# DCDmllm/AnyEdit

Measured on AMD Instinct MI355X. Metric: edited-images/sec @512x512, 50 DDIM steps, higher is better.
Workload: dtype bf16; 1 GPU; configs[1]: AnySD (SD-1.5 UNet in=8 + task embedding/expert adapters) 512x512 bf16, 50 DDIM steps, batch=4/GPU, 3-branch CFG (UNet batch 12); images_per_gpu=4, ddim_steps=50, cfg_branches=3, hip_graph=True, parallelism=dp1 (image-sharded, no data-path collective)

## Files before the change

anyedit_amd/_lib.py:

```python
import ctypes
import os

import torch

_HERE = os.path.dirname(os.path.abspath(__file__))
LIB_PATH = os.environ.get("AE_LIB_PATH") or os.path.join(_HERE, "libanyedit_hip.so")

c_void_p, c_int, c_long, c_float = ctypes.c_void_p, ctypes.c_int, ctypes.c_long, ctypes.c_float

SIGNATURES = {
    "ae_version": [],
    "ae_last_error": [],
    "ae_device_arch": [ctypes.c_char_p, c_int],
    "ae_device_info": [ctypes.POINTER(c_int), ctypes.POINTER(c_long), ctypes.POINTER(c_int)],
    "ae_gemm_bf16": [c_void_p, c_long, c_void_p, c_long, c_int, c_void_p, c_long, c_void_p, c_long, c_int, c_int, c_int,
                     c_void_p, c_void_p, c_long, c_void_p, c_long, c_int, c_int, c_int, c_void_p, c_void_p],
    "ae_conv3x3_workspace_floats": [c_int, c_int, c_int, c_int, c_int, c_int, c_int],
    "ae_conv3x3_bf16": [c_void_p, c_void_p, c_void_p, c_void_p, c_long, c_void_p, c_void_p, c_int, c_int, c_int, c_int, c_int,
                        c_int, c_int, c_int, c_void_p, c_void_p, c_int, c_void_p],
    "ae_conv3x3_up2_bf16": [c_void_p, c_void_p, c_void_p, c_void_p, c_int, c_int, c_int, c_int, c_int, c_void_p, c_void_p],
    "ae_gemm_plan": [c_int] * 8 + [ctypes.POINTER(c_int)],
    "ae_conv3x3_plan": [c_int] * 11 + [ctypes.POINTER(c_int)],
    "ae_conv3x3_up2_plan": [c_int] * 6 + [ctypes.POINTER(c_int)],
    "ae_groupnorm_rows_per_chunk": [c_int, c_int],
# ... 86 lines not shown
    "ae_clip_embed_bf16": [c_void_p, c_int, c_void_p, c_void_p, c_void_p, c_int, c_int, c_int, c_int, c_int, c_void_p],
    "ae_bias_act_f32_bf16": [c_void_p, c_long, c_void_p, c_void_p, c_long, c_long, c_int, c_int, c_void_p],
    "ae_clip_pool_eos_bf16": [c_void_p, c_int, c_void_p, c_void_p, c_int, c_int, c_int, c_long, c_void_p],
    "ae_clip_patch_rows_bf16": [c_void_p, c_int, c_void_p, c_int, c_int, c_int, c_int, c_int, c_int, c_float, c_void_p, c_void_p, c_void_p],
    "ae_clip_vision_embed_ln_bf16": [c_void_p, c_long, c_void_p, c_void_p, c_void_p, c_void_p, c_void_p, c_int, c_int, c_int, c_float, c_void_p],
    "ae_clip_vision_pool_ln_bf16": [c_void_p, c_long, c_void_p, c_void_p, c_void_p, c_int, c_int, c_float, c_void_p],
    "ae_dino_embed_bf16": [c_void_p, c_long, c_void_p, c_void_p, c_void_p, c_void_p, c_int, c_int, c_int, c_void_p],
    "ae_swiglu_f32_bf16": [c_void_p, c_long, c_void_p, c_void_p, c_long, c_long, c_int, c_void_p],
    "ae_swin_window_attn_bf16": [c_void_p, c_long, c_void_p, c_void_p, c_void_p, c_long, c_int, c_int, c_int, c_int, c_int, c_int, c_int, c_float, c_void_p],
    "ae_swin_merge_ln_bf16": [c_void_p, c_void_p, c_void_p, c_void_p, c_int, c_int, c_int, c_int, c_float, c_void_p],
    "ae_scale_residual_f32_bf16": [c_void_p, c_long, c_void_p, c_void_p, c_void_p, c_long, c_void_p, c_long, c_long, c_int, c_void_p],
    "ae_biattn_split_rows": [c_int],
    "ae_biattn_workspace_bytes": [c_int, c_int, c_int, c_int, c_int],
    "ae_biattn_bf16": [c_void_p, c_long] * 4 + [c_void_p, c_void_p] + [c_void_p, c_long] * 2 + [c_int] * 5 + [c_float, c_void_p, c_long, c_void_p],
    "ae_attn_masked_short_bf16": [c_void_p] * 5 + [c_int] * 4 + [c_long] * 12 + [c_float, c_void_p],
    "ae_contrastive_bf16": [c_void_p, c_long, c_void_p, c_void_p, c_void_p, c_long, c_void_p] + [c_int] * 5 + [c_void_p],
    "ae_topk_rows_max_n": [],
    "ae_topk_rows_f32": [c_void_p, c_long, c_void_p, c_int, c_int, c_int, c_void_p],
    "ae_gdino_proposals_f32": [c_void_p, ctypes.POINTER(c_int), ctypes.POINTER(c_int), c_int, c_void_p, c_void_p, c_int, c_int, c_void_p],
    "ae_gdino_query_sine": [c_void_p, c_void_p, c_void_p, c_void_p, c_long, c_int, c_int, c_int, c_void_p],
    "ae_gdino_box_refine_f32": [c_void_p, c_long, c_void_p, c_void_p, c_void_p, c_void_p, c_void_p, c_long, c_int, c_void_p],
    "ae_gdino_text_spans": [c_void_p, c_int, c_int, c_int, c_int] + [c_long] * 8 + [c_void_p, c_void_p, c_void_p, c_void_p],
    "ae_bert_embed_ln_bf16": [c_void_p, c_void_p, c_void_p] + [c_void_p] * 6 + [c_int] * 6 + [c_float, c_void_p],
    "ae_attn_span_short_bf16": [c_void_p] * 5 + [c_int] * 4 + [c_long] * 12 + [c_float, c_void_p],
    "ae_gdino_level_geometry": [c_void_p, c_int, c_int, c_int, ctypes.POINTER(c_int), ctypes.POINTER(c_int), c_int, c_float, c_float, c_void_p, c_void_p, c_void_p,
                                c_void_p, c_int, c_void_p],
    "ae_gdino_neck_groupnorm_workspace_floats": [c_int, c_int],
    "ae_gdino_neck_groupnorm": [c_void_p, c_long, c_void_p, c_void_p, c_float, c_void_p, c_long, c_long, c_int, c_int, c_void_p, c_void_p],
    "ae_gdino_ground": [c_void_p, c_void_p, c_float, c_float, c_void_p, c_void_p, c_void_p, c_void_p, c_void_p, c_int, c_int, c_int, c_void_p],
    "ae_hed_stem_bf16": [c_void_p, c_int, c_long, c_long, c_long, c_long, c_void_p, c_void_p, c_void_p, c_void_p, c_int, c_int, c_int, c_int, c_void_p],
    "ae_relu_bf16": [c_void_p, c_long, c_void_p],
    "ae_hed_tail_bf16": [c_void_p, c_void_p, c_void_p, c_void_p, c_void_p, c_int, c_int, c_int, c_int, c_void_p],
    "ae_hed_fuse": [c_void_p] * 7 + [c_int] * 4 + [c_void_p],
}
_RESTYPES = {"ae_last_error": ctypes.c_char_p, "ae_groupnorm_workspace_floats": c_long, "ae_conv3x3_workspace_floats": c_long,
             "ae_groupnorm_bwd_workspace_floats": c_long, "ae_attn_fp8_workspace_bytes": c_long, "ae_attn_bwd_workspace_floats": c_long,
             "ae_biattn_workspace_bytes": c_long, "ae_gdino_neck_groupnorm_workspace_floats": c_long}


class AnyEditHipError(RuntimeError):
    pass


def _load():
    if not os.path.exists(LIB_PATH):
        raise ImportError(
            f"{LIB_PATH} is missing: the HIP extension is REQUIRED (no CPU/eager fallback exists). "
            "Build it with `python -c 'import __graft_entry__ as g; g.build()'` or `python anyedit_amd/build.py`.")
    lib = ctypes.CDLL(LIB_PATH)
    for name, argtypes in SIGNATURES.items():
        fn = getattr(lib, name)
        fn.argtypes = argtypes
        fn.restype = _RESTYPES.get(name, c_int)
    return lib


lib = _load()


def check(rc, what=""):
    if rc != 0:
        msg = lib.ae_last_error()
        raise AnyEditHipError(f"{what} failed (rc={rc}): {msg.decode() if msg else ''}")


def device_arch():
# ... 4 lines not shown
```

anyedit_amd/build.py:

```python
import hashlib
import os
import shutil
import subprocess
import sys

HERE = os.path.dirname(os.path.abspath(__file__))
CSRC = os.path.join(HERE, "csrc")
LIB = os.path.join(HERE, "libanyedit_hip.so")
SOURCES = ["c_api.hip", "gemm_conv.hip", "gemm_rowpanel.hip", "ff_fused.hip", "attention.hip", "attention_fast.hip", "attention_fp8.hip", "attention_bwd.hip", "norm.hip", "elementwise.hip", "backward.hip", "gate.hip", "expert_kv.hip", "msda.hip",
           "sam_decoder.hip", "clip_text.hip", "clip_vision.hip", "dino_vision.hip", "swin.hip", "gdino_encoder.hip", "gdino_decoder.hip", "gdino_text.hip", "gdino_neck.hip", "hed.hip"]
EXTRA = {"gemm_conv.hip": ["-fno-slp-vectorize"], "gemm_rowpanel.hip": ["-fno-slp-vectorize"], "ff_fused.hip": ["-fno-slp-vectorize"], "attention.hip": ["-ffinite-math-only"],
         "attention_fast.hip": ["-ffinite-math-only", "-fno-slp-vectorize"], "attention_fp8.hip": ["-ffinite-math-only"],
         "attention_bwd.hip": ["-ffinite-math-only"], "clip_text.hip": ["-ffinite-math-only"]}
FLAGS = ["--offload-arch=gfx950", "-O3", "-std=c++17", "-fPIC", "-fno-gpu-rdc", "-Wno-unused-result"]


def _hipcc():
    for c in (shutil.which("hipcc"), "/opt/rocm/bin/hipcc"):
        if c and os.path.exists(c):
            return c
    raise RuntimeError("hipcc not found: the HIP extension cannot be built")


def _digest():
    h = hashlib.sha256()
    for name in sorted(os.listdir(CSRC)):
        with open(os.path.join(CSRC, name), "rb") as f:
            h.update(name.encode() + f.read())
    h.update((" ".join(FLAGS) + repr(sorted(EXTRA.items()))).encode())
    return h.hexdigest()


def build_library(force=False, verbose=True, variant=None, extra_flags=None):
    lib = LIB if variant is None else os.path.join(HERE, f"libanyedit_hip_{variant}.so")
    extra = {k: list(v) for k, v in EXTRA.items()}
    for k, v in (extra_flags or {}).items():
        if k not in SOURCES:
            raise ValueError(f"{k} is not a source of the library")
        extra[k] = extra.get(k, []) + list(v)
    stamp = lib + ".sha256"
    dig = _digest() if variant is None else None
    if not force and dig is not None and os.path.exists(lib) and os.path.exists(stamp) and open(stamp).read().strip() == dig:
        return lib
    objdir = os.path.join(HERE, "build" if variant is None else f"build_{variant}")
# ... 38 lines not shown
```

anyedit_amd/csrc/norm.hip:

```cpp
#include "common.hpp"
#include <stdlib.h>

#ifndef GN_CS_U
#define GN_CS_U 4
#endif

namespace {

constexpr int GN_MAXR = 8;

struct GNArgs {
    const bf16_t* x; const bf16_t* x2;
    int C1;
    const float* gamma; const float* beta;
    bf16_t* y;
    float* part;
    float* coef;
    int B, HW, C, groups, rows_per_chunk, nchunk, act;
    float eps;
    float* stat;
    const bf16_t* dy; bf16_t* dx; bf16_t* dx2;
    float* part2;
    float* coef2;
    int* counters;
// ... 997 lines not shown
        AE_REQUIRE(HW % 32 == 0, "ae_groupnorm_nhwc_bf16: producer statistics are kept per 32-row slab: HW=%d must be a multiple of 32", HW);
        AE_REQUIRE((x2 == nullptr) == (colstats2 == nullptr), "ae_groupnorm_nhwc_bf16: statistics are needed for both sources of a concat input");
        AE_REQUIRE(((uintptr_t)colstats & 7) == 0 && ((uintptr_t)colstats2 & 7) == 0, "ae_groupnorm_nhwc_bf16: colstats alignment");
        AE_REQUIRE((long)(HW / 32) * (C / groups) < (1L << 20), "ae_groupnorm_nhwc_bf16: %ld slab sums per group exceed the 2^20 the statistics fold indexes exactly", (long)(HW / 32) * (C / groups));
        p.cs1 = colstats; p.cs2 = colstats2;
        hipLaunchKernelGGL(gn_finalize_cs_kernel, dim3(groups, B), dim3(256), 0, s, p);
        int rc0 = ae_check_launch("ae_groupnorm_nhwc_bf16(finalize from producer statistics)");
        if (rc0) return rc0;
        hipLaunchKernelGGL(gn_apply_kernel<false>, grid, dim3(threads), 0, s, p);
        return ae_check_launch("ae_groupnorm_nhwc_bf16(apply)");
    }
    static const int slab = getenv("AE_GN_SLAB") ? atoi(getenv("AE_GN_SLAB")) : 1;
    if (slab && HW <= 256) {
        const int cpg = C / groups;
        const int gp = (cpg % 8 == 0) ? 1 : ((2 * cpg) % 8 == 0 ? 2 : ((4 * cpg) % 8 == 0 ? 4 : 0));
        bool done = false;
        if (gp == 1 && groups % 1 == 0) done = launch_gn_slab<1>(p, cpg, s);
        else if (gp == 2 && groups % 2 == 0) done = launch_gn_slab<2>(p, cpg, s);
        else if (gp == 4 && groups % 4 == 0) done = launch_gn_slab<4>(p, cpg, s);
        if (done) return ae_check_launch("ae_groupnorm_nhwc_bf16(slab)");
    }
    hipLaunchKernelGGL(gn_stats_kernel, grid, dim3(threads), (size_t)(threads / ncc) * 2 * C * sizeof(float), s, p);
    int rc = ae_check_launch("ae_groupnorm_nhwc_bf16(stats)");
    if (rc) return rc;
    if (p.counters) {
        hipLaunchKernelGGL(gn_apply_kernel<false>, grid, dim3(threads), 0, s, p);
        return ae_check_launch("ae_groupnorm_nhwc_bf16(apply)");
    }
    hipLaunchKernelGGL(gn_finalize_kernel, dim3(B), dim3(1024), 0, s, p);
    rc = ae_check_launch("ae_groupnorm_nhwc_bf16(finalize)");
    if (rc) return rc;
    hipLaunchKernelGGL(gn_apply_kernel<false>, grid, dim3(threads), 0, s, p);
    return ae_check_launch("ae_groupnorm_nhwc_bf16(apply)");
}

extern "C" int ae_layernorm_bf16(const void* x, const float* gamma, const float* beta, void* y, int M, int C, float eps,
                                 void* stream) {
    AE_REQUIRE(x && gamma && beta && y, "ae_layernorm_bf16: null pointer");
    AE_REQUIRE(M > 0 && C > 0 && C % 8 == 0, "ae_layernorm_bf16: C=%d must be a positive multiple of 8", C);
    AE_REQUIRE(C <= 4096, "ae_layernorm_bf16: C=%d > 4096 unsupported", C);
    AE_REQUIRE(((uintptr_t)x & 15) == 0 && ((uintptr_t)y & 15) == 0, "ae_layernorm_bf16: 16-byte alignment");
    dim3 grid((M + 3) / 4), block(256);
    const int ncc = C / 8;
    hipStream_t s = (hipStream_t)stream;
    static const int rows_kernel = getenv("AE_LN_ROWS") ? atoi(getenv("AE_LN_ROWS")) : 1;
    const bool al16 = (((uintptr_t)gamma | (uintptr_t)beta) & 15) == 0;
    if (rows_kernel && al16 && ncc % 5 == 0 && (ncc == 40 || ncc == 80 || ncc == 160 || ncc == 320)) {
        const int L = ncc / 5, rpb = 4 * (64 / L);
        dim3 g2((unsigned)((M + rpb - 1) / rpb));
        if (L == 8) hipLaunchKernelGGL((layernorm_rows_kernel<8, 5>), g2, block, 0, s, (const bf16_t*)x, gamma, beta, (bf16_t*)y, M, C, eps);
        else if (L == 16) hipLaunchKernelGGL((layernorm_rows_kernel<16, 5>), g2, block, 0, s, (const bf16_t*)x, gamma, beta, (bf16_t*)y, M, C, eps);
        else if (L == 32) hipLaunchKernelGGL((layernorm_rows_kernel<32, 5>), g2, block, 0, s, (const bf16_t*)x, gamma, beta, (bf16_t*)y, M, C, eps);
        else hipLaunchKernelGGL((layernorm_rows_kernel<64, 5>), g2, block, 0, s, (const bf16_t*)x, gamma, beta, (bf16_t*)y, M, C, eps);
        return ae_check_launch("ae_layernorm_bf16");
    }
    if (ncc <= 64) hipLaunchKernelGGL(layernorm_kernel<1>, grid, block, 0, s, (const bf16_t*)x, gamma, beta, (bf16_t*)y, M, C, eps);
    else if (ncc <= 128) hipLaunchKernelGGL(layernorm_kernel<2>, grid, block, 0, s, (const bf16_t*)x, gamma, beta, (bf16_t*)y, M, C, eps);
    else if (ncc <= 192) hipLaunchKernelGGL(layernorm_kernel<3>, grid, block, 0, s, (const bf16_t*)x, gamma, beta, (bf16_t*)y, M, C, eps);
    else hipLaunchKernelGGL(layernorm_kernel<8>, grid, block, 0, s, (const bf16_t*)x, gamma, beta, (bf16_t*)y, M, C, eps);
    return ae_check_launch("ae_layernorm_bf16");
}

extern "C" int ae_layernorm_window_supported(int C) {
    const int ncc = C / 8;
    return C % 8 == 0 && (ncc == 40 || ncc == 80 || ncc == 160 || ncc == 320);
}
// ... 134 lines not shown
```

anyedit_amd/ldm/modules/attention.py:

```python
import os

import torch
import torch.nn as nn

from anyedit_amd import ops
from anyedit_amd.ldm.util import default, exists
from anyedit_amd.ldm.modules.diffusionmodules.util import Linear, Conv2d, LayerNorm, checkpoint

BF16 = torch.bfloat16
_FF_TAIL = os.environ.get("AE_FF_TAIL", "1") != "0"
_SEG2_160 = os.environ.get("AE_ATTN_SEG2_160", "1") != "0"


def zero_module(module):
    for p in module.parameters():
        p.detach().zero_()
    return module


class _GN6(nn.GroupNorm):

    def _affine(self):
        if ops.cache_stale(self, "_pk", self.weight, self.bias):
            self._pk = (self.weight.detach().float().contiguous(), self.bias.detach().float().contiguous())
# ... 275 lines not shown


class SpatialTransformer(nn.Module):

    def __init__(self, in_channels, n_heads, d_head, depth=1, dropout=0., context_dim=None, disable_self_attn=False,
                 use_linear=False, use_checkpoint=True):
        super().__init__()
        if exists(context_dim) and not isinstance(context_dim, list):
            context_dim = [context_dim] * depth
        if context_dim is None:
            context_dim = [None] * depth
        self.in_channels = in_channels
        inner_dim = n_heads * d_head
        self.norm = Normalize(in_channels)
        if not use_linear:
            self.proj_in = Conv2d(in_channels, inner_dim, kernel_size=1, stride=1, padding=0)
        else:
            self.proj_in = Linear(in_channels, inner_dim)
        self.transformer_blocks = nn.ModuleList(
            [BasicTransformerBlock(inner_dim, n_heads, d_head, dropout=dropout, context_dim=context_dim[d],
                                   disable_self_attn=disable_self_attn, checkpoint=use_checkpoint) for d in range(depth)])
        if not use_linear:
            self.proj_out = zero_module(Conv2d(inner_dim, in_channels, kernel_size=1, stride=1, padding=0))
        else:
            self.proj_out = zero_module(Linear(in_channels, inner_dim))
        self.use_linear = use_linear

    def rows(self, x, B, H, W, context_rows=None, kv_cache=None, colstats=None, out_colstats=None):
        if isinstance(context_rows, (list, tuple)):
            ctxs = list(context_rows)
        else:
            ctxs = [context_rows] * len(self.transformer_blocks)
        N = H * W
        h = self.norm.rows(x, B, N, colstats=colstats)
        pin = self.proj_in._packed()
        M, Ci = h.shape[0], pin["w"].shape[0]
        st = None
        if self.transformer_blocks[0].wants_rowstats(M, Ci) and ops.ln_fold_plan(M, Ci, h.shape[1], ops.EPI_NONE, 1):
            st = ops.rowstats_buffer(M, Ci, h.device)
        h = ops.gemm(h, pin["w"], pin["b"], rowstats=st)
        pout = self.proj_out._packed()
        last = len(self.transformer_blocks) - 1
        tail_ok = self.transformer_blocks[last].takes_tail(M, Ci) and pout["w"].shape == (Ci, Ci) and x.shape[1] == Ci
        for i, blk in enumerate(self.transformer_blocks):
            tail = (pout["w"], pout["b"], x, out_colstats) if (tail_ok and i == last) else None
            h = blk.rows(h, B, N, context_rows=ctxs[i], kv_cache=kv_cache, rowstats=st if i == 0 else None, tail=tail)
        if tail_ok:
            return h
        return ops.gemm(h, pout["w"], pout["b"], residual=x, colstats=out_colstats)

    def forward(self, x, context=None):
        B, C, H, W = x.shape
        if isinstance(context, list):
            ctx = [None if c is None else c.reshape(-1, c.shape[-1]).to(BF16).contiguous() for c in context]
        else:
            ctx = None if context is None else context.reshape(-1, context.shape[-1]).to(BF16).contiguous()
        y = self.rows(ops.nchw_to_rows(x), B, H, W, context_rows=ctx)
        return ops.rows_to_nchw(y, B, H, W, out_dtype=x.dtype)
```

anyedit_amd/ops.py:

```python
import torch

import collections
import ctypes
import os
import threading

from ._lib import lib, check as _check

BF16 = torch.bfloat16
EPI_NONE, EPI_GELU, EPI_GEGLU, EPI_SILU, EPI_RELU = 0, 1, 2, 3, 4


def _s():
    return torch.cuda.current_stream().cuda_stream


def _p(t):
    return None if t is None else t.data_ptr()


_live = threading.local()


def _tmp(t):
# ... 460 lines not shown

def _gn_counters(device, B):
    if not _GN_TAIL:
        return None
    key = (device, torch.cuda.current_stream(device).cuda_stream)
    c = _GN_COUNTERS.get(key)
    if c is None or c.numel() < B:
        c = _GN_COUNTERS[key] = torch.zeros(max(B, 256), dtype=torch.int32, device=device)
    return c


def groupnorm(x, gamma, beta, B, HW, eps, silu=False, groups=32, x2=None, out=None, stat_out=None, colstats=None, colstats2=None):
    if _TAPE is not None and _TAPE.active:
        return _TAPE.groupnorm(x, gamma, beta, B, HW, eps, silu=silu, groups=groups, x2=x2, out=out)
    _chk(x, BF16, "groupnorm.x", 2)
    C1 = x.shape[1]
    C = C1 + (x2.shape[1] if x2 is not None else 0)
    if not x.is_contiguous() or (x2 is not None and not x2.is_contiguous()):
        raise ValueError("groupnorm: inputs must be contiguous")
    if out is None:
        out = torch.empty(B * HW, C, dtype=BF16, device=x.device)
    if colstats is not None and (x2 is None) != (colstats2 is None):
        colstats = colstats2 = None
    if colstats is not None:
        for t, c, n in ((colstats, C1, "colstats"), (colstats2, C - C1, "colstats2")):
            if t is not None and (t.dtype != torch.float32 or tuple(t.shape) != (B * HW // 32, c, 2) or not t.is_contiguous() or HW % 32):
                raise ValueError(f"groupnorm: {n} must be a contiguous fp32 [{B * HW // 32}, {c}, 2] buffer (HW % 32 == 0), got {tuple(t.shape)}")
    nws = int(lib.ae_groupnorm_workspace_floats(B, HW, C, groups))
    ws = torch.empty(nws, dtype=torch.float32, device=x.device)
    check(lib.ae_groupnorm_nhwc_bf16(_p(x), _p(x2), C1, _p(gamma), _p(beta), _p(out), B, HW, C, groups, eps,
                                     1 if silu else 0, _p(ws), _p(_gn_counters(x.device, B)), _p(stat_out), _p(colstats), _p(colstats2), _s()),
          "ae_groupnorm_nhwc_bf16")
    return out


def layernorm(x, gamma, beta, eps=1e-5, out=None):
    if _TAPE is not None and _TAPE.active:
        return _TAPE.layernorm(x, gamma, beta, eps=eps, out=out)
    _chk(x, BF16, "layernorm.x", 2)
    if not x.is_contiguous():
        raise ValueError("layernorm: x must be contiguous")
    M, C = x.shape
    if out is None:
        out = torch.empty_like(x)
    check(lib.ae_layernorm_bf16(_p(x), _p(gamma), _p(beta), _p(out), M, C, eps, _s()), "ae_layernorm_bf16")
    return out


def attention(q, k, v, B, H, Nq, Nk, D, scale, q_strides, k_strides, v_strides, out=None, rel_h=None, rel_w=None,
              kH=0, kW=0, key_mask=None, out_scale=None, accumulate=False, seg2=None, lse=None, lse2=None, o_strides=None):
    if _TAPE is not None and _TAPE.active:
        return _TAPE.attention(q, k, v, B, H, Nq, Nk, D, scale, q_strides, k_strides, v_strides, out=out, key_mask=key_mask,
                               out_scale=out_scale, accumulate=accumulate, seg2=seg2, rel_h=rel_h)
    if out is None:
        out = torch.empty(B, Nq, H * D, dtype=BF16, device=q.device)
    if o_strides is None:
        o_strides = (Nq * H * D, D, H * D)
    if seg2 is not None:
        k2, v2, Nk2, k2_strides, v2_strides, scale2 = seg2
        seg_args = (_p(k2), _p(v2), Nk2, *k2_strides, *v2_strides, _p(scale2))
    else:
        seg_args = (None, None, 0, 0, 0, 0, 0, 0, 0, None)
    check(lib.ae_attn_fwd_bf16(_p(q), _p(k), _p(v), _p(out), B, H, Nq, Nk, D, *q_strides, *k_strides, *v_strides, *o_strides,
                               scale, _p(rel_h), _p(rel_w), kH, kW, _p(key_mask), _p(out_scale), 1 if accumulate else 0,
                               *seg_args, _p(lse), _p(lse2), _s()), "ae_attn_fwd_bf16")
    return out
# ... 1597 lines not shown


def _gemm_ln_label(_r, a, w, bias, residual, epilogue, out, M, N, K, rowstats_out, ln_stats, nparts, ln_colsum, eps):
    nb = 2 * (M * K + N * K) + _r.numel() * 2 + (2 * M * N if residual is not None else 0)
    tag = "rowstats" if rowstats_out is not None else "LNfold"
    p = gemm_plan(M, N, K, epilogue, ln_mode=1 if rowstats_out is not None else 2)
    if p.rowpanel:
        return f"gemm_rowpanel_kernel<K=320,{tag}{',geglu' if epilogue == EPI_GEGLU else ''}>|M={M} N={N}", 2.0 * M * N * K, nb
    return f"gemm_kernel<{plan_label(p)},dense,{tag}>|M={M} N={N} K={K}", 2.0 * M * N * K, float(nb)


def _up2_label(_r, x, w4, bias, B, H, W, **_):
    y = _r[0]
    Cout, Cin = w4.shape[1], x.shape[1]
    tl = plan_label(up2_plan(B, H, W, Cin, Cout, _.get("colstats") is not None))
    nb = 2 * (x.numel() + 16 * Cin * Cout) + 2 * y.numel()
    return f"gemm_kernel<{tl},conv3x3,up2x2>|M={y.shape[0]} Cin={Cin} Cout={Cout}", 2.0 * y.shape[0] * Cout * 4 * Cin, float(nb)


conv3x3_up2 = _wrap_profiled(conv3x3_up2, _up2_label)
ff_fused = _wrap_profiled(ff_fused, lambda _r, x, gamma, beta, eps, w1, b1, w2img, b2, residual=None, out=None, w3=None, b3=None, residual3=None, colstats=None: (
    f"ff_fused_kernel<C=320{',proj_out' if w3 is not None else ''}>|M={x.shape[0]} H={w1.shape[0] // 2}",
    2.0 * x.shape[0] * x.shape[1] * (3 * (w1.shape[0] // 2) + (x.shape[1] if w3 is not None else 0)),
    float(2 * (x.numel() * (2 + (residual is not None and residual is not x) + (residual3 is not None)) + w1.numel() + w2img.numel() + (w3.numel() if w3 is not None else 0))),
    2 if colstats is not None else 1))
_ln_gemm_fused = _wrap_profiled(_ln_gemm_launch, _ln_gemm_label)
_gemm_ln_launch = _wrap_profiled(_gemm_ln_launch, _gemm_ln_label)
gemm = _wrap_profiled(gemm, _gemm_label)
attention_fp8 = _wrap_profiled(attention_fp8, _attn8_label)
conv3x3 = _wrap_profiled(conv3x3, _conv_label)
attention = _wrap_profiled(attention, _attn_label)
groupnorm = _wrap_profiled(groupnorm, _gn_label)
layernorm = _wrap_profiled(layernorm, _ln_label)
expert_kv = _wrap_profiled(expert_kv, lambda _r, x, W, experts, tokens: (
    f"expert_kv_fwd_kernel|rows={x.shape[0]} N={W.shape[1]} Dc={W.shape[2]}", 2.0 * x.shape[0] * W.shape[1] * W.shape[2], 4.0 * (x.shape[0] // tokens) * W.shape[1] * W.shape[2]))
expert_kv_dgrad = _wrap_profiled(expert_kv_dgrad, lambda _r, dy, W, experts, tokens: (
    f"expert_kv_dgrad_kernel|rows={dy.shape[0]} N={W.shape[1]} Dc={W.shape[2]}", 2.0 * dy.shape[0] * W.shape[1] * W.shape[2], 4.0 * (dy.shape[0] // tokens) * W.shape[1] * W.shape[2]))
expert_kv_wgrad = _wrap_profiled(expert_kv_wgrad, lambda _r, dy, x, experts, tokens, n_experts, out=None: (
    f"expert_kv_wgrad_kernel|rows={dy.shape[0]} N={dy.shape[1]} Dc={x.shape[1]} E={n_experts}", 2.0 * dy.shape[0] * dy.shape[1] * x.shape[1], 4.0 * n_experts * dy.shape[1] * x.shape[1]))
hed_stem = _wrap_profiled(hed_stem, lambda _r, x, norm, w, bias, out=None: (
    f"hed_stem_kernel<{'u8' if x.dtype == torch.uint8 else 'f32'}>|M={_r[0].shape[0]} C1={_r[0].shape[1]}", 2.0 * 27 * _r[0].numel(),
    float(x.numel() * x.element_size() + 2 * _r[0].numel())))
relu_ = _wrap_profiled(relu_, lambda _r, x: (f"relu_bf16_kernel|n={x.numel()}", 0.0, 4.0 * x.numel()))
hed_tail = _wrap_profiled(hed_tail, lambda _r, y, wp, bp, B, H, W, pool=True, proj=None, pooled=None: (
    f"hed_tail_kernel<{'pool' if pool else 'last'}>|M={y.shape[0]} C={y.shape[1]}", 2.0 * y.numel(),
    float(2 * y.numel() + 4 * _r[0].numel() + (2 * _r[1].numel() if pool else 0))))
hed_fuse = _wrap_profiled(hed_fuse, lambda _r, sides, invert=True, out=None, logits=None, want_logits=False: (
    f"hed_fuse_kernel|B={sides[0].shape[0]} {sides[0].shape[-2]}x{sides[0].shape[-1]}", 0.0,
    float(4 * sum(s.numel() for s in sides) + sides[0].numel() * (1 + 4 * (want_logits or logits is not None)))))
```

include/anyedit_hip.h:

```cpp
#ifndef ANYEDIT_HIP_H
#define ANYEDIT_HIP_H

#ifdef __cplusplus
extern "C" {
#endif

#define AE_OK 0
#define AE_ERR_ARG (-1)
#define AE_ERR_LAUNCH (-2)
#define AE_ERR_UNSUPPORTED (-3)

#define AE_EPI_NONE 0
#define AE_EPI_GELU 1
#define AE_EPI_GEGLU 2
#define AE_EPI_SILU 3
#define AE_EPI_RELU 4

int ae_version(void);
const char* ae_last_error(void);
int ae_device_arch(char* buf, int n);
int ae_device_info(int* cus, long* hbm_bytes, int* clock_khz);

int ae_gemm_bf16(const void* A, long lda, const void* A2, long lda2, int Ksplit, const void* W, long ldw, void* C, long ldc,
                 int M, int N, int K, const float* bias, const void* residual, long ldr, const float* addvec, long addvec_ld,
// ... 3 lines not shown
int ae_ln_gemm_bf16(const void* A, long lda, const void* W, long ldw, void* C, long ldc, int M, int N, int K, const float* bias,
                    const void* residual, long ldr, const float* ln_gamma, const float* ln_beta, float ln_eps, int epilogue,
                    float* colstats , void* stream);

int ae_gemm_ln_plan(int M, int N, int K, int epilogue, int mode);
int ae_gemm_ln_bf16(const void* A, long lda, const void* W, long ldw, void* C, long ldc, int M, int N, int K, const float* bias,
                    const void* residual, long ldr, int epilogue, float* rowstats_out, const float* ln_stats, int ln_parts,
                    const float* ln_colsum, float ln_eps, void* stream);

int ae_ff_fused_supported(int M, int C, int H);
int ae_ff_fused_bf16(const void* X, long ldx, const float* ln_gamma, const float* ln_beta, float ln_eps, const void* W1, long ldw1, const float* b1,
                     const void* W2img, const float* b2, const void* residual, long ldr, const void* W3, long ldw3, const float* b3,
                     const void* residual3, long ldr3, float* colstats, void* Y, long ldy, int M, int C, int H, void* stream);

long ae_conv3x3_workspace_floats(int B, int H, int W, int Cin, int Cout, int stride, int upsample2x);
int ae_conv3x3_bf16(const void* x, const void* w, const float* bias, const float* addvec, long addvec_ld, const void* residual,
                    void* y, int B, int H, int W, int Cin, int Cout, int stride, int upsample2x, int out_f32, float* workspace,
                    float* colstats , int k_order, void* stream);

int ae_conv3x3_up2_bf16(const void* x, const void* w4, const float* bias, void* y, int B, int H, int W, int Cin, int Cout,
                        float* colstats, void* stream);

#define AE_PLAN_INTS 19
int ae_gemm_plan(int M, int N, int K, int epilogue, int Ksplit, int out_f32, int colstats, int ln_mode, int* plan);
int ae_conv3x3_plan(int B, int H, int W, int Cin, int Cout, int stride, int upsample2x, int out_f32, int workspace, int colstats, int k_order,
                    int* plan);
int ae_conv3x3_up2_plan(int B, int H, int W, int Cin, int Cout, int colstats, int* plan);

int ae_groupnorm_rows_per_chunk(int HW, int C);
long ae_groupnorm_workspace_floats(int B, int HW, int C, int groups);
int ae_groupnorm_nhwc_bf16(const void* x, const void* x2, int C1, const float* gamma, const float* beta, void* y, int B, int HW,
                           int C, int groups, float eps, int act, float* workspace, int* counters, float* stat_out,
                           const float* colstats, const float* colstats2, void* stream);

int ae_layernorm_bf16(const void* x, const float* gamma, const float* beta, void* y, int M, int C, float eps, void* stream);

int ae_attn_fwd_bf16(const void* q, const void* k, const void* v, void* out, int B, int H, int Nq, int Nk, int D,
                     long q_sb, long q_sh, long q_sn, long k_sb, long k_sh, long k_sn, long v_sb, long v_sh, long v_sn,
                     long o_sb, long o_sh, long o_sn, float scale, const float* rel_h, const float* rel_w, int kH, int kW,
                     const unsigned char* key_mask, const float* out_scale, int accumulate, const void* k2, const void* v2,
                     int Nk2, long k2_sb, long k2_sh, long k2_sn, long v2_sb, long v2_sh, long v2_sn, const float* scale2,
                     float* lse, float* lse2, void* stream);
long ae_attn_fp8_workspace_bytes(int B, int H, int Nq, int Nk, int D);
int ae_attn_fwd_fp8(const void* q, const void* k, const void* v, void* out, int B, int H, int Nq, int Nk, int D, long q_sb, long q_sh,
                    long q_sn, long k_sb, long k_sh, long k_sn, long v_sb, long v_sh, long v_sn, long o_sb, long o_sh, long o_sn,
                    float scale, const float* rel_h, const float* rel_w, int kH, int kW, void* workspace, long workspace_bytes,
                    void* stream);
long ae_attn_bwd_workspace_floats(int B, int H, int Nq, int Nk, int D);
int ae_attn_bwd_bf16(const void* q, const void* k, const void* v, const void* dout, const void* out, const float* lse, float* delta, void* dq,
                     void* dk, void* dv, int B, int H, int Nq, int Nk, int D, long q_sb, long q_sh, long q_sn, long k_sb,
                     long k_sh, long k_sn, long v_sb, long v_sh, long v_sn, long o_sb, long o_sh, long o_sn, long dq_sb,
                     long dq_sh, long dq_sn, long dk_sb, long dk_sh, long dk_sn, long dv_sb, long dv_sh, long dv_sn,
                     float scale, const float* out_scale, int accumulate_dq, float* workspace, void* stream);
long ae_groupnorm_bwd_workspace_floats(int B, int HW, int C, int groups);
int ae_groupnorm_bwd_nhwc_bf16(const void* x, const void* x2, int C1, const float* gamma, const float* beta, const void* dy,
                               void* dx, void* dx2, int B, int HW, int C, int groups, float eps, int act, float* workspace,
                               int* counters, const float* stat_in, int accumulate, void* stream);
int ae_layernorm_bwd_bf16(const void* x, const float* gamma, const void* dy, void* dx, float* row_stat, int M, int C, float eps,
                          int accumulate, void* stream);
int ae_layernorm_param_grad_f32(const void* x, const void* dy, const float* row_stat, float* dgamma, float* dbeta, int M, int C,
                                void* stream);
int ae_add_bf16(const void* a, const void* b, void* y, long n, void* stream);
int ae_axpy_bf16(const void* a, const void* b, float alpha, void* y, long n, void* stream);
int ae_geglu_fwd_bf16(const void* h, void* y, long M, int F, void* stream);
int ae_geglu_bwd_bf16(const void* h, const void* dy, void* dh, long M, int F, void* stream);
int ae_sumpool2x2_bf16(const void* x, void* y, int B, int H, int W, int C, void* stream);
// ... 155 lines not shown
```

Measured before the change: 6.680 edited-images/sec.

## Fuse GroupNorm apply into the proj_in GEMM for K=320 transformer inputs

Splits GroupNorm into a coefficient-only pass that produces per-batch scale/shift, then applies that affine to the A panel in LDS inside a new proj_in GEMM kernel. This removes writing and rereading the normalized activation tensor. The kernel streams weight chunks through an LDS ring and optionally emits rowstats for the next LayerNorm fold. It only covers K=320 (the level-1 blocks) and falls back to the old path otherwise.

Measured after the change: 6.692 edited-images/sec (median of 6 runs). About the same (+0.2%).

```diff
diff --git a/anyedit_amd/_lib.py b/anyedit_amd/_lib.py
--- a/anyedit_amd/_lib.py
+++ b/anyedit_amd/_lib.py
@@ -142,6 +142,10 @@
     "ae_relu_bf16": [c_void_p, c_long, c_void_p],
     "ae_hed_tail_bf16": [c_void_p, c_void_p, c_void_p, c_void_p, c_void_p, c_int, c_int, c_int, c_int, c_void_p],
     "ae_hed_fuse": [c_void_p] * 7 + [c_int] * 4 + [c_void_p],
+    "ae_groupnorm_coef_covers": [c_int] * 5,
+    "ae_groupnorm_coef_f32": [c_void_p, c_void_p, c_void_p, c_int, c_int, c_int, c_int, c_float, c_void_p, c_void_p, c_void_p, c_void_p],
+    "ae_gn_projin_covers": [c_int, c_int, c_int, c_int, c_long],
+    "ae_gn_projin_bf16": [c_void_p, c_long, c_void_p, c_int, c_int, c_void_p, c_long, c_void_p, c_long, c_int, c_int, c_void_p, c_void_p, c_void_p],
 }
 _RESTYPES = {"ae_last_error": ctypes.c_char_p, "ae_groupnorm_workspace_floats": c_long, "ae_conv3x3_workspace_floats": c_long,
              "ae_groupnorm_bwd_workspace_floats": c_long, "ae_attn_fp8_workspace_bytes": c_long, "ae_attn_bwd_workspace_floats": c_long,
diff --git a/anyedit_amd/build.py b/anyedit_amd/build.py
--- a/anyedit_amd/build.py
+++ b/anyedit_amd/build.py
@@ -8,8 +8,8 @@
 CSRC = os.path.join(HERE, "csrc")
 LIB = os.path.join(HERE, "libanyedit_hip.so")
 SOURCES = ["c_api.hip", "gemm_conv.hip", "gemm_rowpanel.hip", "ff_fused.hip", "attention.hip", "attention_fast.hip", "attention_fp8.hip", "attention_bwd.hip", "norm.hip", "elementwise.hip", "backward.hip", "gate.hip", "expert_kv.hip", "msda.hip",
-           "sam_decoder.hip", "clip_text.hip", "clip_vision.hip", "dino_vision.hip", "swin.hip", "gdino_encoder.hip", "gdino_decoder.hip", "gdino_text.hip", "gdino_neck.hip", "hed.hip"]
-EXTRA = {"gemm_conv.hip": ["-fno-slp-vectorize"], "gemm_rowpanel.hip": ["-fno-slp-vectorize"], "ff_fused.hip": ["-fno-slp-vectorize"], "attention.hip": ["-ffinite-math-only"],
+           "sam_decoder.hip", "clip_text.hip", "clip_vision.hip", "dino_vision.hip", "swin.hip", "gdino_encoder.hip", "gdino_decoder.hip", "gdino_text.hip", "gdino_neck.hip", "hed.hip", "level1_edges.hip"]
+EXTRA = {"gemm_conv.hip": ["-fno-slp-vectorize"], "gemm_rowpanel.hip": ["-fno-slp-vectorize"], "level1_edges.hip": ["-fno-slp-vectorize"], "ff_fused.hip": ["-fno-slp-vectorize"], "attention.hip": ["-ffinite-math-only"],
          "attention_fast.hip": ["-ffinite-math-only", "-fno-slp-vectorize"], "attention_fp8.hip": ["-ffinite-math-only"],
          "attention_bwd.hip": ["-ffinite-math-only"], "clip_text.hip": ["-ffinite-math-only"]}
 FLAGS = ["--offload-arch=gfx950", "-O3", "-std=c++17", "-fPIC", "-fno-gpu-rdc", "-Wno-unused-result"]
diff --git a/anyedit_amd/csrc/level1_edges.hip b/anyedit_amd/csrc/level1_edges.hip
--- /dev/null
+++ b/anyedit_amd/csrc/level1_edges.hip
@@ -0,0 +1,257 @@
+#include "common.hpp"
+#include <stdlib.h>
+
+extern "C" int ae_ln_gemm_supported(int M, int N, int K, int epilogue);
+
+namespace {
+
+struct GnProjArgs {
+    const bf16_t* A; const bf16_t* W; bf16_t* C;
+    const float* bias;
+    const float* coef;
+    float* rowstats;
+    int M, N, B, HW;
+    long lda, ldw, ldc;
+};
+
+constexpr int GP_MF = 3;
+constexpr int GP_RG = 4;
+constexpr int GP_NW = 8;
+constexpr int GP_BN = 32;
+constexpr int GP_PAIRS = 3;
+constexpr int GP_BM = GP_RG * GP_MF * 16;
+constexpr int GP_MAXN = 2560;
+constexpr int GP_KS = 10, GP_K = 32 * GP_KS;
+constexpr int GP_NS = 4;
+constexpr int GP_MINHW = 64;
+
+template <int N>
+__device__ __forceinline__ void gp_wait_dma() {
+    asm volatile("s_waitcnt vmcnt(%0)" ::"n"(N) : "memory");
+}
+
+__device__ __forceinline__ int gp_wrow(int i) { return 8 * ((i & 15) >> 2) + 4 * (i >> 4) + (i & 3); }
+
+__device__ __forceinline__ u32x4 gp_apply(u32x4 t, f32x4 sc0, f32x4 sc1, f32x4 sh0, f32x4 sh1) {
+    u32x4 w;
+    w.x = pack_bf16x2(bf16lo(t.x) * sc0[0] + sh0[0], bf16hi(t.x) * sc0[1] + sh0[1]);
+    w.y = pack_bf16x2(bf16lo(t.y) * sc0[2] + sh0[2], bf16hi(t.y) * sc0[3] + sh0[3]);
+    w.z = pack_bf16x2(bf16lo(t.z) * sc1[0] + sh1[0], bf16hi(t.z) * sc1[1] + sh1[1]);
+    w.w = pack_bf16x2(bf16lo(t.w) * sc1[2] + sh1[2], bf16hi(t.w) * sc1[3] + sh1[3]);
+    return w;
+}
+
+__global__ __launch_bounds__(64 * GP_NW, 2) void l1_gn_projin_kernel(const GnProjArgs p) {
+    constexpr int KS = GP_KS, K = GP_K, ROWB = 2 * K, CHUNKB = GP_BN * ROWB, PIECES = CHUNKB / 1024;
+    constexpr int PPW = 2 * PIECES / GP_NW;
+    constexpr int APW = 6 * PIECES / GP_NW;
+    static_assert((2 * PIECES) % GP_NW == 0 && (6 * PIECES) % GP_NW == 0, "pieces must split evenly over the waves");
+    static_assert(GP_BM == 6 * GP_BN && GP_PAIRS == 3, "the A panel is staged through the six chunk slots of the ring");
+    __shared__ __attribute__((aligned(16))) char smem[2 * GP_PAIRS * CHUNKB + GP_MAXN * 4];
+    float* const sbias = reinterpret_cast<float*>(smem + 2 * GP_PAIRS * CHUNKB);
+    __shared__ __attribute__((aligned(16))) float scoef[GP_NS][2][K];
+    __shared__ __attribute__((aligned(8))) f32x2 sred[2][2][GP_RG][GP_MF][16];
+
+    const int tid = threadIdx.x, lane = tid & 63;
+    const int wave = __builtin_amdgcn_readfirstlane(tid >> 6);
+    const int rg = wave & 3, half = wave >> 2;
+    const int l15 = lane & 15, g = lane >> 4;
+    const int m0 = blockIdx.x * GP_BM + rg * (GP_MF * 16);
+    const int lds0 = (int)(uintptr_t)((__attribute__((address_space(3))) char*)smem);
+
+    const __amdgpu_buffer_rsrc_t rsW = __builtin_amdgcn_make_buffer_rsrc(const_cast<bf16_t*>(p.W), 0, (int)((long)p.N * p.ldw * 2), 0x00020000);
+    int dma_off[PPW];
+#pragma unroll
+    for (int j = 0; j < PPW; ++j) {
+        const int q = wave + GP_NW * j;
+        const int o = (q % PIECES) * 1024 + lane * 16;
+        const int i = o / ROWB, pp = (o - i * ROWB) >> 4;
+        dma_off[j] = ((q / PIECES) * GP_BN + gp_wrow(i)) * (int)p.ldw * 2 + ((pp & ~7) | ((pp ^ (i >> 1)) & 7)) * 16;
+    }
+    const int npairs = p.N / (2 * GP_BN);
+    const int pair_stride = 2 * GP_BN * (int)p.ldw * 2;
+    auto issue = [&](int pi) {
+        const int slot = lds0 + (pi % GP_PAIRS) * 2 * CHUNKB;
+        const int soff = pi * pair_stride;
+#pragma unroll
+        for (int j = 0; j < PPW; ++j) ae_dma16(rsW, slot + (wave + GP_NW * j) * 1024, dma_off[j], soff);
+    };
+
+    {
+        const __amdgpu_buffer_rsrc_t rsA = __builtin_amdgcn_make_buffer_rsrc(const_cast<bf16_t*>(p.A), 0, (int)((long)p.M * p.lda * 2), 0x00020000);
+        const int base = blockIdx.x * GP_BM * (int)p.lda * 2;
+#pragma unroll
+        for (int j = 0; j < APW; ++j) {
+            const int q = wave + GP_NW * j;
+            const int o = (q % PIECES) * 1024 + lane * 16;
+            const int i = o / ROWB, pp = (o - i * ROWB) >> 4;
+            ae_dma16(rsA, lds0 + q * 1024, base + ((q / PIECES) * GP_BN + i) * (int)p.lda * 2 + ((pp & ~7) | ((pp ^ (i >> 1)) & 7)) * 16, 0);
+        }
+    }
+    for (int i = tid; i < p.N; i += 64 * GP_NW) sbias[i] = p.bias ? p.bias[i] : 0.f;
+    const int b0 = (blockIdx.x * GP_BM) / p.HW;
+    for (int i = tid; i < GP_NS * 2 * K; i += 64 * GP_NW) {
+        const int sb = i / (2 * K), j = i - sb * (2 * K);
+        (&scoef[0][0][0])[i] = p.coef[(long)min(b0 + sb, p.B - 1) * (2 * K) + j];
+    }
+    gp_wait_dma<0>();
+    __syncthreads();
+
+    if (tid < 12 * (K / 8)) {
+        const int c = tid % (K / 8), r0 = tid / (K / 8);
+        auto piece = [&](int j) {
+            const int rl = r0 + 12 * j, i = rl & 31;
+            return reinterpret_cast<u32x4*>(smem + (rl >> 5) * CHUNKB + i * ROWB + (((c & ~7) | ((c ^ (i >> 1)) & 7)) << 4));
+        };
+        const int blk0 = blockIdx.x * GP_BM;
+        if (blk0 + GP_BM <= p.M && (blk0 + GP_BM - 1) / p.HW == b0) {
+            u32x4 v[GP_BM / 12];
+#pragma unroll
+            for (int j = 0; j < GP_BM / 12; ++j) v[j] = *piece(j);
+            const float* cs = &scoef[0][0][0] + 8 * c;
+            const f32x4 sc0 = *reinterpret_cast<const f32x4*>(cs), sc1 = *reinterpret_cast<const f32x4*>(cs + 4);
+            const f32x4 sh0 = *reinterpret_cast<const f32x4*>(cs + K), sh1 = *reinterpret_cast<const f32x4*>(cs + K + 4);
+#pragma unroll
+            for (int j = 0; j < GP_BM / 12; ++j) *piece(j) = gp_apply(v[j], sc0, sc1, sh0, sh1);
+        } else {
+            int grow = blk0 + r0;
+            int bound = (min(grow, p.M - 1) / p.HW + 1) * p.HW;
+            const float* cs = &scoef[min(grow, p.M - 1) / p.HW - b0][0][0] + 8 * c;
+            f32x4 sc0 = *reinterpret_cast<const f32x4*>(cs), sc1 = *reinterpret_cast<const f32x4*>(cs + 4);
+            f32x4 sh0 = *reinterpret_cast<const f32x4*>(cs + K), sh1 = *reinterpret_cast<const f32x4*>(cs + K + 4);
+#pragma unroll
+            for (int j = 0; j < GP_BM / 12; ++j) {
+                const bool ok = grow < p.M;
+                if (ok && grow >= bound) {
+                    bound += p.HW;
+                    cs += 2 * K;
+                    sc0 = *reinterpret_cast<const f32x4*>(cs); sc1 = *reinterpret_cast<const f32x4*>(cs + 4);
+                    sh0 = *reinterpret_cast<const f32x4*>(cs + K); sh1 = *reinterpret_cast<const f32x4*>(cs + K + 4);
+                }
+                u32x4* const pc = piece(j);
+                const u32x4 w = gp_apply(*pc, sc0, sc1, sh0, sh1);
+                *pc = ok ? w : (u32x4){0u, 0u, 0u, 0u};
+                grow += 12;
+            }
+        }
+    }
+    __syncthreads();
+    u32x4 af[GP_MF][KS];
+#pragma unroll
+    for (int f = 0; f < GP_MF; ++f) {
+        const int rl = rg * (GP_MF * 16) + 16 * f + l15;
+        const int i = rl & 31;
+        const char* base = smem + (rl >> 5) * CHUNKB + i * ROWB;
+#pragma unroll
+        for (int ks = 0; ks < KS; ++ks) {
+            const int c16 = 4 * ks + g;
+            af[f][ks] = *reinterpret_cast<const u32x4*>(base + (((c16 & ~7) | ((c16 ^ (i >> 1)) & 7)) << 4));
+        }
+    }
+    __syncthreads();
+    for (int pi = 0; pi < GP_PAIRS - 1 && pi < npairs; ++pi) issue(pi);
+
+    int woff[KS];
+#pragma unroll
+    for (int ks = 0; ks < KS; ++ks) {
+        const int c16 = 4 * ks + g;
+        woff[ks] = l15 * ROWB + (((c16 & ~7) | ((c16 ^ (l15 >> 1)) & 7)) << 4);
+    }
+    int coff[GP_MF];
+    bool rok[GP_MF];
+#pragma unroll
+    for (int f = 0; f < GP_MF; ++f) {
+        const int row = m0 + 16 * f + l15;
+        rok[f] = row < p.M;
+        coff[f] = min(row, p.M - 1) * (int)p.ldc + 8 * g;
+    }
+    const bool rs = p.rowstats != nullptr;
+
+    for (int pi = 0; pi < npairs; ++pi) {
+        if (pi + 1 < npairs) gp_wait_dma<PPW>();
+        else gp_wait_dma<0>();
+        __builtin_amdgcn_s_barrier();
+        asm volatile("" ::: "memory");
+        const int c = 2 * pi + half;
+        const int n0 = c * GP_BN;
+        if (pi + GP_PAIRS - 1 < npairs) issue(pi + GP_PAIRS - 1);
+        if (rs && pi > 0 && half == 0 && g == 0) {
+#pragma unroll
+            for (int f = 0; f < GP_MF; ++f) {
+                const f32x2 a0 = sred[(pi - 1) & 1][0][rg][f][l15], a1 = sred[(pi - 1) & 1][1][rg][f][l15];
+                if (rok[f]) *reinterpret_cast<f32x2*>(p.rowstats + ((long)(m0 + 16 * f + l15) * (p.N >> 6) + (pi - 1)) * 2) = (f32x2){a0[0] + a1[0], a0[1] + a1[1]};
+            }
+        }
+
+        const char* slot = smem + ((pi % GP_PAIRS) * 2 + half) * CHUNKB;
+        f32x4 acc[GP_MF][2];
+#pragma unroll
+        for (int f = 0; f < GP_MF; ++f) acc[f][0] = acc[f][1] = (f32x4){0.f, 0.f, 0.f, 0.f};
+#pragma unroll
+        for (int ks = 0; ks < KS; ++ks) {
+#pragma unroll
+            for (int nf = 0; nf < 2; ++nf) {
+                const bf16x8_t wf = as_bf16x8(*reinterpret_cast<const u32x4*>(slot + woff[ks] + nf * 16 * ROWB));
+#pragma unroll
+                for (int f = 0; f < GP_MF; ++f) acc[f][nf] = __builtin_amdgcn_mfma_f32_16x16x32_bf16(wf, as_bf16x8(af[f][ks]), acc[f][nf], 0, 0, 0);
+            }
+        }
+
+        const f32x4 b0v = *reinterpret_cast<const f32x4*>(sbias + n0 + 8 * g), b1v = *reinterpret_cast<const f32x4*>(sbias + n0 + 8 * g + 4);
+        bf16_t* const cb = p.C + n0;
+#pragma unroll
+        for (int f = 0; f < GP_MF; ++f) {
+            const float o0 = acc[f][0][0] + b0v[0], o1 = acc[f][0][1] + b0v[1], o2 = acc[f][0][2] + b0v[2], o3 = acc[f][0][3] + b0v[3];
+            const float o4 = acc[f][1][0] + b1v[0], o5 = acc[f][1][1] + b1v[1], o6 = acc[f][1][2] + b1v[2], o7 = acc[f][1][3] + b1v[3];
+            const u32x4 pk = {pack_bf16x2(o0, o1), pack_bf16x2(o2, o3), pack_bf16x2(o4, o5), pack_bf16x2(o6, o7)};
+            if (rok[f]) *reinterpret_cast<u32x4*>(cb + coff[f]) = pk;
+            const uint32_t w4[4] = {pk.x, pk.y, pk.z, pk.w};
+            float ps = 0.f, pq = 0.f;
+#pragma unroll
+            for (int e = 0; e < 4; ++e) {
+                const float a = bf16lo(w4[e]), c2 = bf16hi(w4[e]);
+                ps += a + c2;
+                pq += a * a + c2 * c2;
+            }
+            ps += __shfl_xor(ps, 16, 64); pq += __shfl_xor(pq, 16, 64);
+            ps += __shfl_xor(ps, 32, 64); pq += __shfl_xor(pq, 32, 64);
+            if (g == 0) sred[pi & 1][half][rg][f][l15] = (f32x2){ps, pq};
+        }
+    }
+    if (rs) {
+        __syncthreads();
+        if (half == 0 && g == 0) {
+#pragma unroll
+            for (int f = 0; f < GP_MF; ++f) {
+                const f32x2 a0 = sred[(npairs - 1) & 1][0][rg][f][l15], a1 = sred[(npairs - 1) & 1][1][rg][f][l15];
+                if (rok[f]) *reinterpret_cast<f32x2*>(p.rowstats + ((long)(m0 + 16 * f + l15) * (p.N >> 6) + (npairs - 1)) * 2) = (f32x2){a0[0] + a1[0], a0[1] + a1[1]};
+            }
+        }
+    }
+}
+
+}
+
+extern "C" int ae_gn_projin_covers(int B, int HW, int N, int K, long ld) {
+    static const int on = getenv("AE_L1_PROJIN") ? atoi(getenv("AE_L1_PROJIN")) : 1;
+    if (!on || B <= 0 || HW < GP_MINHW || (long)B * HW >= (1L << 30) || K != GP_K || ld < K || ld < N || ld % 8) return 0;
+    const int M = B * HW;
+    if (!ae_ln_gemm_supported(M, N, K, 0)) return 0;
+    if (((long)M + GP_BM) * ld * 2 >= (1L << 30) || (long)N * ld * 2 >= (1L << 30)) return 0;
+    return 1;
+}
+
+extern "C" int ae_gn_projin_bf16(const void* x, long ldx, const float* coef, int B, int HW, const void* W, long ldw, void* C, long ldc, int N, int K,
+                                 const float* bias, float* rowstats_out, void* stream) {
+    AE_REQUIRE(x && coef && W && C, "ae_gn_projin_bf16: null pointer");
+    const long ldmax = ldx > ldc ? (ldx > ldw ? ldx : ldw) : (ldc > ldw ? ldc : ldw);
+    AE_REQUIRE(ldx >= K && ldw >= K && ldc >= N && ldx % 8 == 0 && ldw % 8 == 0 && ldc % 8 == 0, "ae_gn_projin_bf16: row strides must cover the rows and keep 16-byte alignment");
+    AE_REQUIRE(ae_gn_projin_covers(B, HW, N, K, ldmax), "ae_gn_projin_bf16: B=%d HW=%d N=%d K=%d ld=%ld is outside the envelope (ae_gn_projin_covers)", B, HW, N, K, ldmax);
+    AE_REQUIRE(((uintptr_t)x & 15) == 0 && ((uintptr_t)W & 15) == 0 && ((uintptr_t)C & 15) == 0 && ((uintptr_t)coef & 15) == 0 && ((uintptr_t)rowstats_out & 7) == 0,
+               "ae_gn_projin_bf16: pointer alignment");
+    GnProjArgs a{};
+    a.A = (const bf16_t*)x; a.W = (const bf16_t*)W; a.C = (bf16_t*)C; a.bias = bias; a.coef = coef; a.rowstats = rowstats_out;
+    a.M = B * HW; a.N = N; a.B = B; a.HW = HW; a.lda = ldx; a.ldw = ldw; a.ldc = ldc;
+    hipLaunchKernelGGL(l1_gn_projin_kernel, dim3((unsigned)((a.M + GP_BM - 1) / GP_BM)), dim3(64 * GP_NW), 0, (hipStream_t)stream, a);
+    return ae_check_launch("ae_gn_projin_bf16");
+}
diff --git a/anyedit_amd/csrc/norm.hip b/anyedit_amd/csrc/norm.hip
--- a/anyedit_amd/csrc/norm.hip
+++ b/anyedit_amd/csrc/norm.hip
@@ -1053,6 +1053,46 @@
     if (rc) return rc;
     hipLaunchKernelGGL(gn_apply_kernel<false>, grid, dim3(threads), 0, s, p);
     return ae_check_launch("ae_groupnorm_nhwc_bf16(apply)");
+}
+
+extern "C" int ae_groupnorm_coef_covers(int B, int HW, int C, int groups, int has_colstats) {
+    if (B <= 0 || B > 65535 || HW <= 0 || C <= 0 || groups <= 0 || groups > 64 || C % groups || C % 8 || C > 8192) return 0;
+    if (has_colstats) return (HW % 32 == 0 && (long)(HW / 32) * (C / groups) < (1L << 20)) ? 1 : 0;
+    static const int slab = getenv("AE_GN_SLAB") ? atoi(getenv("AE_GN_SLAB")) : 1;
+    return (!slab || HW > 256) ? 1 : 0;
+}
+
+extern "C" int ae_groupnorm_coef_f32(const void* x, const float* gamma, const float* beta, int B, int HW, int C, int groups, float eps, float* workspace,
+                                     const float* colstats, float* coef_out, void* stream) {
+    AE_REQUIRE(gamma && beta && coef_out && (x || colstats), "ae_groupnorm_coef_f32: null pointer");
+    AE_REQUIRE(B > 0 && B <= 65535 && HW > 0 && C > 0 && groups > 0 && groups <= 64 && C % groups == 0 && C % 8 == 0 && C <= 8192,
+               "ae_groupnorm_coef_f32: bad shape B=%d HW=%d C=%d groups=%d", B, HW, C, groups);
+    AE_REQUIRE(((uintptr_t)x & 15) == 0 && ((uintptr_t)coef_out & 15) == 0 && ((uintptr_t)workspace & 15) == 0 && ((uintptr_t)colstats & 7) == 0, "ae_groupnorm_coef_f32: alignment");
+    GNArgs p{};
+    p.x = (const bf16_t*)x; p.C1 = C; p.gamma = gamma; p.beta = beta;
+    p.B = B; p.HW = HW; p.C = C; p.groups = groups; p.eps = eps;
+    p.rows_per_chunk = ae_groupnorm_rows_per_chunk(HW, C);
+    p.nchunk = (HW + p.rows_per_chunk - 1) / p.rows_per_chunk;
+    p.part = workspace;
+    p.coef = coef_out;
+    hipStream_t s = (hipStream_t)stream;
+    if (colstats) {
+        AE_REQUIRE(HW % 32 == 0 && (long)(HW / 32) * (C / groups) < (1L << 20), "ae_groupnorm_coef_f32: producer statistics are kept per 32-row slab (HW=%d), at most 2^20 slab sums per group", HW);
+        p.cs1 = colstats;
+        hipLaunchKernelGGL(gn_finalize_cs_kernel, dim3(groups, B), dim3(256), 0, s, p);
+        return ae_check_launch("ae_groupnorm_coef_f32(finalize from producer statistics)");
+    }
+    AE_REQUIRE(x && workspace, "ae_groupnorm_coef_f32: the statistics pass needs x and a workspace of ae_groupnorm_workspace_floats");
+    const int ncc = C / 8;
+    int rpp = 256 / ncc;
+    if (rpp < 1) rpp = 1;
+    int threads = ncc * rpp;
+    if (threads < 64) threads = 64;
+    hipLaunchKernelGGL(gn_stats_kernel, dim3(p.nchunk, B), dim3(threads), (size_t)(threads / ncc) * 2 * C * sizeof(float), s, p);
+    const int rc = ae_check_launch("ae_groupnorm_coef_f32(stats)");
+    if (rc) return rc;
+    hipLaunchKernelGGL(gn_finalize_kernel, dim3(B), dim3(1024), 0, s, p);
+    return ae_check_launch("ae_groupnorm_coef_f32(finalize)");
 }
 
 extern "C" int ae_layernorm_bf16(const void* x, const float* gamma, const float* beta, void* y, int M, int C, float eps,
diff --git a/anyedit_amd/ldm/modules/attention.py b/anyedit_amd/ldm/modules/attention.py
--- a/anyedit_amd/ldm/modules/attention.py
+++ b/anyedit_amd/ldm/modules/attention.py
@@ -331,13 +331,13 @@
         else:
             ctxs = [context_rows] * len(self.transformer_blocks)
         N = H * W
-        h = self.norm.rows(x, B, N, colstats=colstats)
         pin = self.proj_in._packed()
-        M, Ci = h.shape[0], pin["w"].shape[0]
+        M, Ci = x.shape[0], pin["w"].shape[0]
         st = None
-        if self.transformer_blocks[0].wants_rowstats(M, Ci) and ops.ln_fold_plan(M, Ci, h.shape[1], ops.EPI_NONE, 1):
-            st = ops.rowstats_buffer(M, Ci, h.device)
-        h = ops.gemm(h, pin["w"], pin["b"], rowstats=st)
+        if self.transformer_blocks[0].wants_rowstats(M, Ci) and ops.ln_fold_plan(M, Ci, x.shape[1], ops.EPI_NONE, 1):
+            st = ops.rowstats_buffer(M, Ci, x.device)
+        g, b = self.norm._affine()
+        h = ops.groupnorm_proj_in(x, g, b, self.norm.eps, pin["w"], pin["b"], B, N, groups=self.norm.num_groups, colstats=colstats, rowstats=st)
         pout = self.proj_out._packed()
         last = len(self.transformer_blocks) - 1
         tail_ok = self.transformer_blocks[last].takes_tail(M, Ci) and pout["w"].shape == (Ci, Ci) and x.shape[1] == Ci
diff --git a/anyedit_amd/ops.py b/anyedit_amd/ops.py
--- a/anyedit_amd/ops.py
+++ b/anyedit_amd/ops.py
@@ -516,6 +516,64 @@
                                      1 if silu else 0, _p(ws), _p(_gn_counters(x.device, B)), _p(stat_out), _p(colstats), _p(colstats2), _s()),
           "ae_groupnorm_nhwc_bf16")
     return out
+
+
+def groupnorm_coef_ok(B, HW, C, groups=32, colstats=None):
+    if _TAPE is not None and _TAPE.active:
+        return False
+    return bool(lib.ae_groupnorm_coef_covers(B, HW, C, groups, 1 if colstats is not None else 0))
+
+
+def groupnorm_coef(x, gamma, beta, B, HW, eps, groups=32, colstats=None, out=None):
+    _no_tape("groupnorm_coef")
+    _chk(x, BF16, "groupnorm_coef.x", 2)
+    C = x.shape[1]
+    if x.shape[0] != B * HW or not x.is_contiguous():
+        raise ValueError(f"groupnorm_coef: x must be contiguous [B*HW, C] = [{B * HW}, C], got {tuple(x.shape)}")
+    if colstats is not None and (colstats.dtype != torch.float32 or tuple(colstats.shape) != (B * HW // 32, C, 2) or not colstats.is_contiguous() or HW % 32):
+        raise ValueError(f"groupnorm_coef: colstats must be a contiguous fp32 [{B * HW // 32}, {C}, 2] buffer (HW % 32 == 0), got {tuple(colstats.shape)}")
+    coef = _target(out, torch.float32, (B, 2, C), "groupnorm_coef.out") if out is not None else torch.empty(B, 2, C, dtype=torch.float32, device=x.device)
+    ws = None
+    if colstats is None:
+        ws = torch.empty(int(lib.ae_groupnorm_workspace_floats(B, HW, C, groups)), dtype=torch.float32, device=x.device)
+    check(lib.ae_groupnorm_coef_f32(_p(x), _p(gamma), _p(beta), B, HW, C, groups, eps, _p(ws), _p(colstats), _p(coef), _s()), "ae_groupnorm_coef_f32")
+    return coef
+
+
+def gn_proj_in_ok(x, w, B, HW, out=None):
+    if not _ROWPANEL or (_TAPE is not None and _TAPE.active) or x.dim() != 2 or w.dim() != 2 or x.shape[0] != B * HW or x.shape[1] != w.shape[1]:
+        return False
+    ts = [x, w] + ([out] if out is not None else [])
+    if not all(t.dtype == BF16 and t.data_ptr() % 16 == 0 and t.stride(0) % 8 == 0 and t.stride(1) == 1 for t in ts):
+        return False
+    return bool(lib.ae_gn_projin_covers(B, HW, w.shape[0], w.shape[1], max([t.stride(0) for t in ts] + [w.shape[0]])))
+
+
+def gn_proj_in(x, coef, w, bias, B, HW, out=None, rowstats=None):
+    _no_tape("gn_proj_in")
+    _chk(x, BF16, "gn_proj_in.x", 2)
+    _chk(w, BF16, "gn_proj_in.w", 2)
+    M, K = x.shape
+    N = w.shape[0]
+    if coef.dtype != torch.float32 or tuple(coef.shape) != (B, 2, K) or not coef.is_contiguous() or M != B * HW or w.shape[1] != K:
+        raise ValueError(f"gn_proj_in: x is {tuple(x.shape)} = [B*HW, K], w {tuple(w.shape)}; coef must be the contiguous fp32 [{B}, 2, {K}] of groupnorm_coef")
+    if out is None:
+        out = torch.empty(M, N, dtype=BF16, device=x.device)
+    _chk(out, BF16, "gn_proj_in.out", 2)
+    if bias is not None:
+        _chk(bias, torch.float32, "gn_proj_in.bias", 1)
+    if rowstats is not None and (rowstats.dtype != torch.float32 or tuple(rowstats.shape) != (M, N // 64, 2) or not rowstats.is_contiguous()):
+        raise ValueError(f"gn_proj_in: rowstats must be a contiguous fp32 [{M}, {N // 64}, 2] buffer (rowstats_buffer)")
+    check(lib.ae_gn_projin_bf16(_p(x), x.stride(0), _p(coef), B, HW, _p(w), w.stride(0), _p(out), out.stride(0), N, K, _p(bias), _p(rowstats), _s()),
+          "ae_gn_projin_bf16")
+    return out
+
+
+def groupnorm_proj_in(x, gamma, beta, eps, w, bias, B, HW, groups=32, colstats=None, rowstats=None):
+    if gn_proj_in_ok(x, w, B, HW) and groupnorm_coef_ok(B, HW, x.shape[1], groups, colstats):
+        coef = groupnorm_coef(x, gamma, beta, B, HW, eps, groups=groups, colstats=colstats)
+        return gn_proj_in(x, coef, w, bias, B, HW, rowstats=rowstats)
+    return gemm(groupnorm(x, gamma, beta, B, HW, eps, groups=groups, colstats=colstats), w, bias, rowstats=rowstats)
 
 
 def layernorm(x, gamma, beta, eps=1e-5, out=None):
@@ -2179,6 +2237,12 @@
 attention = _wrap_profiled(attention, _attn_label)
 groupnorm = _wrap_profiled(groupnorm, _gn_label)
 layernorm = _wrap_profiled(layernorm, _ln_label)
+groupnorm_coef = _wrap_profiled(groupnorm_coef, lambda _r, x, gamma, beta, B, HW, eps, groups=32, colstats=None, out=None: (
+    f"groupnorm_coef(stats)|rows={x.shape[0]} C={x.shape[1]}", 0.0,
+    float(8 * (x.shape[0] // 32) * x.shape[1] if colstats is not None else 2 * x.numel()) + 4.0 * _r.numel(), 1 if colstats is not None else 2))
+gn_proj_in = _wrap_profiled(gn_proj_in, lambda _r, x, coef, w, bias, B, HW, out=None, rowstats=None: (
+    f"l1_gn_projin_kernel<K=320{',rowstats' if rowstats is not None else ''}>|M={x.shape[0]} N={w.shape[0]}", 2.0 * x.shape[0] * w.shape[0] * w.shape[1],
+    float(2 * (x.numel() + w.numel() + _r.numel()) + 4 * coef.numel())))
 expert_kv = _wrap_profiled(expert_kv, lambda _r, x, W, experts, tokens: (
     f"expert_kv_fwd_kernel|rows={x.shape[0]} N={W.shape[1]} Dc={W.shape[2]}", 2.0 * x.shape[0] * W.shape[1] * W.shape[2], 4.0 * (x.shape[0] // tokens) * W.shape[1] * W.shape[2]))
 expert_kv_dgrad = _wrap_profiled(expert_kv_dgrad, lambda _r, dy, W, experts, tokens: (
diff --git a/include/anyedit_hip.h b/include/anyedit_hip.h
--- a/include/anyedit_hip.h
+++ b/include/anyedit_hip.h
@@ -59,6 +59,14 @@
 int ae_groupnorm_nhwc_bf16(const void* x, const void* x2, int C1, const float* gamma, const float* beta, void* y, int B, int HW,
                            int C, int groups, float eps, int act, float* workspace, int* counters, float* stat_out,
                            const float* colstats, const float* colstats2, void* stream);
+
+int ae_groupnorm_coef_covers(int B, int HW, int C, int groups, int has_colstats);
+int ae_groupnorm_coef_f32(const void* x, const float* gamma, const float* beta, int B, int HW, int C, int groups, float eps, float* workspace,
+                          const float* colstats, float* coef_out, void* stream);
+
+int ae_gn_projin_covers(int B, int HW, int N, int K, long ld);
+int ae_gn_projin_bf16(const void* x, long ldx, const float* coef, int B, int HW, const void* W, long ldw, void* C, long ldc, int N, int K,
+                      const float* bias, float* rowstats_out, void* stream);
 
 int ae_layernorm_bf16(const void* x, const float* gamma, const float* beta, void* y, int M, int C, float eps, void* stream);
 
```
